# facebookresearch/goliath

Measured on NVIDIA B200. Metric: rendered megapixels/sec (fwd+bwd) RGCA head 300k Gaussians, higher is better.
Workload: dtype f32

## Files before the change

goliath_b200/_lib.py:

```python
import ctypes
import os

import torch

_HERE = os.path.dirname(os.path.abspath(__file__))
LIB_PATH = os.path.join(_HERE, "libgoliath_b200.so")
_lib = None

_vp, _i, _f, _i64, _sz = ctypes.c_void_p, ctypes.c_int, ctypes.c_float, ctypes.c_int64, ctypes.c_size_t

SIGNATURES = {
    "gb_version": (_i, []),
    "gb_launch_count": (ctypes.c_ulonglong, []),
    "gb_launch_count_reset": (None, []),
    "gb_sg_evaluate_fwd": (_i, [_vp] * 7 + [_i] * 4 + [_vp]),
    "gb_sg_evaluate_bwd": (_i, [_vp] * 10 + [_i] * 4 + [_vp]),
    "gb_project_gaussians_fwd": (_i, [_i, _vp, _vp, _f, _vp, _vp, _f, _f, _f, _f, _i, _i, _i, _f] + [_vp] * 7 + [_vp]),
    "gb_project_gaussians_bwd": (_i, [_i, _vp, _vp, _f, _vp, _vp, _f, _f] + [_vp] * 13 + [_vp]),
    "gb_cumsum_workspace_bytes": (_sz, [_i]),
    "gb_cumsum_i32": (_i, [_i, _vp, _vp, _vp, _vp]),
    "gb_map_gaussian_to_intersects": (_i, [_i, _vp, _vp, _vp, _vp, _i, _i, _i, _vp, _vp, _vp]),
    "gb_sort_workspace_bytes": (_sz, [_i64]),
    "gb_sort_intersects": (_i, [_i64, _vp, _vp, _vp, _vp, _i, _vp, _vp]),
    "gb_get_tile_bin_edges": (_i, [_i64, _vp, _vp, _vp]),
    "gb_rasterize_fwd": (_i, [_i, _i, _i, _i] + [_vp] * 10 + [_vp]),
    "gb_rasterize_bwd": (_i, [_i, _i, _i, _i] + [_vp] * 15 + [_vp]),
    "gb_pack_records": (_i, [_i64, _i] + [_vp] * 6 + [_vp]),
    "gb_tile_order": (_i, [_i, _vp, _vp, _vp]),
    "gb_pack_records_fused": (_i, [_i64] + [_vp] * 8 + [_vp]),
    "gb_pack_records_fused_dn": (_i, [_i64] + [_vp] * 9 + [_vp]),
    "gb_map_gaussian_to_intersects_dn": (_i, [_i, _vp, _vp, _vp, _vp, _i, _i, _i, _i64, _vp, _vp, _vp]),
    "gb_sort_intersects_dn": (_i, [_i64, _vp, _vp, _vp, _vp, _vp, _i, _vp, _vp]),
    "gb_get_tile_bin_edges_dn": (_i, [_i64, _vp, _vp, _vp, _vp, _vp]),
    "gb_get_tile_sort_mode": (_i, []),
    "gb_set_tile_sort_mode": (None, [_i]),
    "gb_get_rank_sort_mode": (_i, []),
    "gb_set_rank_sort_mode": (None, [_i]),
    "gb_bin_tiles_supported": (_i, [_i]),
    "gb_bin_tiles_workspace_bytes": (_sz, [_i, _i, _i64]),
    "gb_bin_tiles_pack": (_i, [_i] + [_vp] * 7 + [_i, _i, _i, _i64] + [_vp, _vp, _i] + [_vp] * 5 + [_vp]),
    "gb_bin_tiles_pack_ev": (_i, [_i] + [_vp] * 7 + [_i, _i, _i, _i64] + [_vp, _vp, _i] + [_vp] * 5 + [_vp, _vp]),
    "gb_tile_schedule_ints": (_i, [_i]),
    "gb_tile_schedule": (_i, [_i, _vp, _vp, _vp]),
    "gb_rasterize_sched_fwd": (_i, [_i, _i, _i] + [_vp] * 7 + [_vp]),
    "gb_rasterize_sched_bwd": (_i, [_i, _i, _i] + [_vp] * 13 + [_vp]),
    "gb_records_widen": (_i, [_i64, _vp, _vp, _vp, _vp]),
    "gb_records_set_colors4": (_i, [_i64, _vp, _vp, _vp, _i, _i64, _vp, _vp]),
    "gb_rasterize_multi_fwd": (_i, [_i, _i, _vp, _vp, _i, _vp, _vp, _vp, _vp]),
    "gb_rasterize_multi_bwd": (_i, [_i, _i, _vp, _vp, _vp, _i] + [_vp] * 9 + [_vp]),
    "gb_colors12_unpack": (_i, [_i64, _i, _vp, _vp, _vp]),
    "gb_records_set_colors": (_i, [_i64] + [_vp] * 5 + [_vp]),
    "gb_splat_grad_unpack": (_i, [_i] + [_vp] * 8 + [_vp]),
    "gb_get_blend_mode": (_i, []),
    "gb_set_blend_mode": (None, [_i]),
    "gb_rasterize_packed_fwd": (_i, [_i, _i, _i] + [_vp] * 7 + [_vp]),
    "gb_rasterize_packed_bwd": (_i, [_i, _i, _i] + [_vp] * 13 + [_vp]),
    "gb_rasterize_ranked_fwd": (_i, [_i, _i, _i] + [_vp] * 8 + [_vp]),
    "gb_rasterize_ranked_bwd": (_i, [_i, _i, _i] + [_vp] * 14 + [_vp]),
    "gb_bin_tiles_ranked": (_i, [_i] + [_vp] * 7 + [_i, _i, _i, _i64] + [_vp, _vp, _i] + [_vp] * 6 + [_vp, _vp]),
    "gb_compute_raydirs_fwd": (_i, [_i, _i, _i] + [_vp] * 5 + [_f] + [_vp] * 3 + [_vp]),
    "gb_compute_raydirs_bwd": (_i, []),
    "gb_mvp_aabb_workspace_bytes": (_sz, [_i, _i]),
    "gb_mvp_compute_aabb": (_i, [_i, _i] + [_vp] * 8 + [_vp]),
    "gb_get_raymarch_mode": (_i, []),
    "gb_set_raymarch_mode": (None, [_i]),
    "gb_mvp_raymarch_fwd": (_i, [_i] * 4 + [_vp, _vp, _f] + [_vp] * 5 + [_i] * 3 + [_vp] + [_i] * 3 + [_vp] * 4
# ... 79 lines not shown
```

goliath_b200/csrc/splat_bin_tiles.cu:

```cuda
#include <stdlib.h>
#include <string.h>

#include "common.cuh"
#include "splat_record.cuh"

extern "C" int gb_tile_order(int num_tiles, const int32_t* tile_bins, int32_t* order, void* stream);
extern "C" int gb_tile_schedule(int num_tiles, const int32_t* tile_bins, int32_t* sched, void* stream);
GB_API int gb_bin_tiles_pack_ev(int G, const float* xys, const float* depths, const int32_t* radii, const float* conics,
                                const float* colors3, const float* opacity, const float* compensation, int img_h,
                                int img_w, int block_width, int64_t cap, int32_t* tile_bins, int32_t* tile_order,
                                int tile_sched, int32_t* gids_sorted, float* records, int32_t* n_out, int32_t* overflow,
                                void* workspace, void* colors_ready, void* stream);

namespace {

constexpr int kRankBlock = 256;
constexpr int kRadix = 256;
constexpr int kRankPasses = 4;
constexpr int kScatItems = 2;
constexpr int kSortThreads = 512;
constexpr int kCopyBatch = 2;
constexpr int kMaxBitmapBytes = 192 * 1024;
constexpr int kMaxSmemTiles = 20 * 1024;

// ... 8 lines not shown
    if (lane >= o) inc += t;
  }
  if (lane == 31) s_warp[warp] = inc;
  __syncthreads();
  if (warp == 0) {
    int w = (lane < (int)(blockDim.x >> 5)) ? s_warp[lane] : 0;
    int winc = w;
#pragma unroll
    for (int o = 1; o < 32; o <<= 1) {
      int t = __shfl_up_sync(0xffffffffu, winc, o);
      if (lane >= o) winc += t;
    }
    s_warp[lane] = winc - w;
    if (lane == 31) s_warp[32] = winc;
  }
  __syncthreads();
  total = s_warp[32];
  const int r = s_warp[warp] + inc - v;
  __syncthreads();
  return r;
}

__device__ __forceinline__ void tile_bbox(float cx, float cy, float radius, int tbx, int tby, int bw, int& x0,
                                          int& y0, int& x1, int& y1) {
  const float fb = (float)bw;
  const float tcx = __fdiv_rn(cx, fb), tcy = __fdiv_rn(cy, fb), tr = __fdiv_rn(radius, fb);
  x0 = min(max(0, __float2int_rz(__fsub_rn(tcx, tr))), tbx);
  x1 = min(max(0, __float2int_rz(__fadd_rn(__fadd_rn(tcx, tr), 1.f))), tbx);
  y0 = min(max(0, __float2int_rz(__fsub_rn(tcy, tr))), tby);
  y1 = min(max(0, __float2int_rz(__fadd_rn(__fadd_rn(tcy, tr), 1.f))), tby);
}

constexpr int kGaussBlock = 1024;
template <int kTileKeys>
__global__ void __launch_bounds__(kGaussBlock) depth_keys_kernel(int G, const float2* __restrict__ xys,
                                                                 const float* __restrict__ depths,
                                                                 const int* __restrict__ radii, int tbx, int tby,
                                                                 int block_width, int smem_tiles,
                                                                 unsigned* __restrict__ keys,
                                                                 unsigned* __restrict__ hist0 ,
                                                                 int* __restrict__ tile_counts,
                                                                 unsigned* __restrict__ key_bits ) {
  constexpr int kItems = kTileKeys / kGaussBlock;
  extern __shared__ int s_cnt[];
  __shared__ unsigned s_hist[kRadix];
  __shared__ unsigned s_or, s_orc, s_max, s_maxc;
  if (threadIdx.x == 0) s_or = s_orc = s_max = s_maxc = 0u;
  if (threadIdx.x < kRadix) s_hist[threadIdx.x] = 0;
  for (int t = threadIdx.x; t < smem_tiles; t += kGaussBlock) s_cnt[t] = 0;
  const int base = blockIdx.x * kTileKeys;
  unsigned k[kItems];
  int r[kItems];
  float2 c[kItems];
#pragma unroll
  for (int j = 0; j < kItems; ++j) {
    const int i = base + j * kGaussBlock + threadIdx.x;
    const bool in = i < G;
    k[j] = in ? __float_as_uint(depths[i]) : 0u;
    r[j] = in ? radii[i] : 0;
    c[j] = in ? xys[i] : make_float2(0.f, 0.f);
  }
  {
    unsigned o = 0u, oc = 0u, mx = 0u, mxc = 0u;
#pragma unroll
    for (int j = 0; j < kItems; ++j)
      if (r[j] > 0) { o |= k[j]; oc |= ~k[j]; mx = max(mx, k[j]); mxc = max(mxc, ~k[j]); }
    o = __reduce_or_sync(0xffffffffu, o);
    oc = __reduce_or_sync(0xffffffffu, oc);
    mx = __reduce_max_sync(0xffffffffu, mx);
    mxc = __reduce_max_sync(0xffffffffu, mxc);
    __syncthreads();
    if ((threadIdx.x & 31) == 0 && (o | oc)) {
      atomicOr(&s_or, o); atomicOr(&s_orc, oc); atomicMax(&s_max, mx); atomicMax(&s_maxc, mxc);
    }
  }
  __syncthreads();
#pragma unroll
  for (int j = 0; j < kItems; ++j) {
    const int i = base + j * kGaussBlock + threadIdx.x;
    if (i >= G) continue;
    keys[i] = k[j];
    atomicAdd(&s_hist[k[j] & 0xffu], 1u);
    if (r[j] > 0) {
      int x0, y0, x1, y1;
      tile_bbox(c[j].x, c[j].y, (float)r[j], tbx, tby, block_width, x0, y0, x1, y1);
      for (int ty = y0; ty < y1; ++ty)
        for (int tx = x0; tx < x1; ++tx) {
          if (smem_tiles) atomicAdd(&s_cnt[ty * tbx + tx], 1);
          else atomicAdd(&tile_counts[ty * tbx + tx], 1);
        }
    }
  }
  __syncthreads();
  if (threadIdx.x == 0 && (s_or | s_orc)) {
    atomicOr(key_bits, s_or); atomicOr(key_bits + 1, s_orc);
    atomicMax(key_bits + 4, s_max); atomicMax(key_bits + 5, s_maxc);
  }
  if (threadIdx.x < kRadix) hist0[(size_t)blockIdx.x * kRadix + threadIdx.x] = s_hist[threadIdx.x];
  for (int t = threadIdx.x; t < smem_tiles; t += kGaussBlock) {
    const int cnt = s_cnt[t];
    if (cnt) atomicAdd(&tile_counts[t], cnt);
  }
}

template <int kItems>
__global__ void __launch_bounds__(kRankBlock) rank_scatter_kernel(
    int n, const unsigned* __restrict__ keys_in, const int* __restrict__ vals_in ,
    unsigned* __restrict__ keys_out , int* __restrict__ vals_out, int shift, int ctas,
    const unsigned* __restrict__ hist_cur ,
    unsigned* __restrict__ hist_next ,
    int* __restrict__ rank_of ) {
  constexpr int kWarps = kRankBlock / 32;
  constexpr int kTile = kRankBlock * kItems;
  __shared__ unsigned s_whist[kWarps][kRadix];
  __shared__ int s_scan[33];
  const int lane = threadIdx.x & 31, warp = threadIdx.x >> 5;

  const int warp_base = blockIdx.x * kTile + warp * (32 * kItems);
  unsigned k[kItems];
  int v[kItems];
#pragma unroll
  for (int j = 0; j < kItems; ++j) {
    const int i = warp_base + j * 32 + lane;
    k[j] = (i < n) ? keys_in[i] : 0xffffffffu;
    v[j] = (i < n) ? (vals_in ? vals_in[i] : i) : 0;
  }

  __shared__ uint4 s_part[2][4][kRadix / 4];
  {
    const int g = threadIdx.x >> 6, c4 = threadIdx.x & 63;
    const uint4* tab = reinterpret_cast<const uint4*>(hist_cur);
// ... 356 lines not shown
    for (int j = 0; j < n; ++j) {
      const unsigned kj = s_k[j];
      r += (kj < ki || (kj == ki && s_id[j] < idi)) ? 1 : 0;
    }
    rank_to_gid[off + r] = idi;
    rank_of[idi] = off + r;
  }
}

__global__ void __launch_bounds__(1024) tile_scan_kernel(int T, long long cap, const int* __restrict__ counts,
                                                         int2* __restrict__ tile_bins, int* __restrict__ cursor,
                                                         int* __restrict__ n_out, int* __restrict__ overflow) {
  __shared__ int s_warp[33];
  int carry = 0;
  for (int base = 0; base < T; base += blockDim.x) {
    const int i = base + threadIdx.x;
    const int v = (i < T) ? counts[i] : 0;
    int total;
    const int ex = block_exclusive_scan(v, s_warp, total);
    if (i < T) {
      const int s = carry + ex;
      cursor[i] = s;
      const int cs = (int)min((long long)s, cap), ce = (int)min((long long)s + v, cap);
      tile_bins[i] = (ce > cs) ? make_int2(cs, ce) : make_int2(0, 0);
    }
    carry += total;
  }
  if (threadIdx.x == 0) {
    if (n_out) *n_out = carry;
    if (overflow && (long long)carry > cap) *overflow = 1;
  }
}

__global__ void __launch_bounds__(kGaussBlock) tile_scatter_kernel(
    int G, const float2* __restrict__ xys, const int* __restrict__ radii, const int* __restrict__ rank_of,
    const float* __restrict__ conics, const float* __restrict__ colors3, const float* __restrict__ depths,
    const float* __restrict__ opacity, const float* __restrict__ comp, int tbx, int tby, int block_width,
    long long cap, int smem_tiles, int* __restrict__ cursor, int* __restrict__ tile_ranks,
    float4* __restrict__ rec_by_rank) {
  extern __shared__ int s_cnt[];
  int* s_base = s_cnt + smem_tiles;
  for (int t = threadIdx.x; t < smem_tiles; t += kGaussBlock) s_cnt[t] = 0;
  const int base = blockIdx.x * (kGaussBlock * kScatItems);
  int rk[kScatItems], r[kScatItems];
  float2 c[kScatItems];
#pragma unroll
  for (int j = 0; j < kScatItems; ++j) {
    const int i = base + j * kGaussBlock + threadIdx.x;
    const bool in = i < G;
    r[j] = in ? radii[i] : 0;
    c[j] = in ? xys[i] : make_float2(0.f, 0.f);
    rk[j] = in ? rank_of[i] : 0;
  }
  __syncthreads();
  unsigned bx[kScatItems], by[kScatItems];
#pragma unroll
  for (int j = 0; j < kScatItems; ++j) {
    const int i = base + j * kGaussBlock + threadIdx.x;
    bx[j] = by[j] = 0u;
    if (r[j] <= 0) continue;
    int x0, y0, x1, y1;
    tile_bbox(c[j].x, c[j].y, (float)r[j], tbx, tby, block_width, x0, y0, x1, y1);
    bx[j] = (unsigned)x0 | ((unsigned)x1 << 16);
    by[j] = (unsigned)y0 | ((unsigned)y1 << 16);
    gb::pack_record_fused(i, xys, conics, colors3, depths, opacity, comp, rec_by_rank + 3 * (size_t)rk[j]);
    for (int ty = y0; ty < y1; ++ty)
      for (int tx = x0; tx < x1; ++tx) {
        if (smem_tiles) {
          atomicAdd(&s_cnt[ty * tbx + tx], 1);
        } else {
          const int pos = atomicAdd(&cursor[ty * tbx + tx], 1);
          if ((long long)pos < cap) tile_ranks[pos] = rk[j];
        }
      }
  }
  if (!smem_tiles) return;
  __syncthreads();
  for (int t = threadIdx.x; t < smem_tiles; t += kGaussBlock) {
    const int cnt = s_cnt[t];
    s_base[t] = cnt ? atomicAdd(&cursor[t], cnt) : 0;
    s_cnt[t] = 0;
  }
  __syncthreads();
#pragma unroll
  for (int j = 0; j < kScatItems; ++j) {
    const int x0 = bx[j] & 0xffffu, x1 = bx[j] >> 16, y0 = by[j] & 0xffffu, y1 = by[j] >> 16;
    for (int ty = y0; ty < y1; ++ty)
      for (int tx = x0; tx < x1; ++tx) {
        const int t = ty * tbx + tx;
        const int pos = s_base[t] + atomicAdd(&s_cnt[t], 1);
        if ((long long)pos < cap) tile_ranks[pos] = rk[j];
      }
  }
}

__global__ void __launch_bounds__(kSortThreads, 3) tile_sort_pack_kernel(
    int words , int chunk , const int* __restrict__ order,
    const int2* __restrict__ tile_bins, const int* __restrict__ tile_ranks, const int* __restrict__ rank_to_gid,
    const float4* __restrict__ rec_by_rank, int* __restrict__ gids_sorted, float4* __restrict__ rec) {
  extern __shared__ unsigned s_bits[];
  __shared__ int s_warp[33];
  const int tile = order ? order[blockIdx.x] : (int)blockIdx.x;
  const int2 range = tile_bins[tile];
  const int n = range.y - range.x;
  if (n <= 0) return;
  for (int w = threadIdx.x; w < words; w += kSortThreads) s_bits[w] = 0u;
  __syncthreads();
  for (int i0 = threadIdx.x; i0 < n; i0 += 4 * kSortThreads) {
    int r[4];
#pragma unroll
    for (int u = 0; u < 4; ++u) {
      const int i = i0 + u * kSortThreads;
      r[u] = (i < n) ? tile_ranks[range.x + i] : -1;
    }
#pragma unroll
    for (int u = 0; u < 4; ++u)
      if (r[u] >= 0) atomicOr(&s_bits[r[u] >> 5], 1u << (r[u] & 31));
  }
  __syncthreads();
  const int w0 = threadIdx.x * chunk, w1 = min(words, w0 + chunk);
  int cnt = 0;
  for (int w = w0; w < w1; ++w) cnt += __popc(s_bits[w]);
  int total;
  int pos = range.x + block_exclusive_scan(cnt, s_warp, total);
// ... 43 lines not shown
  const int tile = order ? order[blockIdx.x] : (int)blockIdx.x;
  const int2 range = tile_bins[tile];
  const int n = range.y - range.x;
  if (n <= 0) return;
  for (int w = threadIdx.x; w < words; w += kSortThreads) s_bits[w] = 0u;
  __syncthreads();
  for (int i0 = threadIdx.x; i0 < n; i0 += 4 * kSortThreads) {
    int r[4];
#pragma unroll
    for (int u = 0; u < 4; ++u) {
      const int i = i0 + u * kSortThreads;
      r[u] = (i < n) ? tile_ranks[range.x + i] : -1;
    }
#pragma unroll
    for (int u = 0; u < 4; ++u)
      if (r[u] >= 0) atomicOr(&s_bits[r[u] >> 5], 1u << (r[u] & 31));
  }
  __syncthreads();
  const int w0 = threadIdx.x * chunk, w1 = min(words, w0 + chunk);
  int cnt = 0;
  for (int w = w0; w < w1; ++w) cnt += __popc(s_bits[w]);
  int total;
  int pos = range.x + block_exclusive_scan(cnt, s_warp, total);
  for (int w = w0; w < w1; ++w) {
    unsigned m = s_bits[w];
    while (m) {
      const int b = __ffs(m) - 1;
      m &= m - 1;
      tile_ranks[pos++] = w * 32 + b;
    }
  }
}

__global__ void __launch_bounds__(256) rec_colors_kernel(int G, const int* __restrict__ radii,
                                                         const int* __restrict__ rank_of,
                                                         const float* __restrict__ colors3,
                                                         const float* __restrict__ depths, float4* __restrict__ rec_by_rank) {
  const int g = blockIdx.x * blockDim.x + threadIdx.x;
  if (g >= G || radii[g] <= 0) return;
  rec_by_rank[3 * (size_t)rank_of[g] + 2] = make_float4(colors3[3 * (size_t)g], colors3[3 * (size_t)g + 1],
                                                       colors3[3 * (size_t)g + 2], depths[g]);
}

__global__ void __launch_bounds__(256) gather_records_kernel(long long cap, const int* __restrict__ n_dev,
                                                             const int* __restrict__ ranks_sorted,
                                                             const int* __restrict__ rank_to_gid,
                                                             const float4* __restrict__ rec_by_rank,
                                                             int* __restrict__ gids_sorted, float4* __restrict__ rec) {
  const long long n = min((long long)*n_dev, cap);
  const long long j = (long long)blockIdx.x * blockDim.x + threadIdx.x;
  if (j >= 3 * n) return;
  const long long i = j / 3;
  const int part = (int)(j - 3 * i);
  const int r = ranks_sorted[i];
  rec[j] = gb::ld_nc_f4(rec_by_rank + 3 * (size_t)r + part);
  if (part == 0) gids_sorted[i] = rank_to_gid[r];
}

struct Layout {
  size_t counts, hist, buckets, sync, zero_bytes, cursor, keys_a, keys_b, vals_a, vals_b, rank_to_gid, rank_of, rec_by_rank,
      tile_ranks, total;
};
inline size_t align256(size_t b) { return (b + 255) & ~(size_t)255; }
inline Layout make_layout(int G, int T, int64_t cap) {
  const int g1 = G > 0 ? G : 1;
  const size_t ctas = (size_t)gb::cdiv(g1, kRankBlock * rank_items(g1));
  const size_t g4 = align256((size_t)g1 * 4);
  Layout l;
  size_t o = 0;
  l.counts = o; o += align256((size_t)T * 4);
  l.hist = o;   o += align256(ctas * kRadix * 4 * kRankPasses);
  l.buckets = o; o += align256((size_t)3 * 2048 * 4);
  l.sync = o;   o += 256;
  l.zero_bytes = o;
  l.cursor = o; o += align256((size_t)T * 4);
  l.keys_a = o; o += g4;
  l.keys_b = o; o += g4;
  l.vals_a = o; o += g4;
  l.vals_b = o; o += g4;
  l.rank_to_gid = o; o += g4;
  l.rank_of = o; o += g4;
  l.rec_by_rank = o; o += align256((size_t)g1 * 48);
  l.tile_ranks = o; o += align256((size_t)(cap > 0 ? cap : 1) * 4);
  l.total = o;
  return l;
}

int g_tile_sort_mode = -1;
int tile_sort_mode() {
  if (g_tile_sort_mode < 0) {
    const char* e = getenv("GOLIATH_B200_TILESORT");
    g_tile_sort_mode = (e && strcmp(e, "fused") == 0) ? 1 : 0;
  }
  return g_tile_sort_mode;
}
int g_rank_sort_mode = -1;
int rank_sort_mode() {
  if (g_rank_sort_mode < 0) {
    const char* e = getenv("GOLIATH_B200_RANKSORT");
    g_rank_sort_mode = !e ? 0 : strcmp(e, "passes") == 0 ? 1 : strcmp(e, "buckets") == 0 ? 2 : 0;
  }
  return g_rank_sort_mode;
}
int sm_count() {
  static int n[64] = {};
  int dev = 0;
  if (cudaGetDevice(&dev) != cudaSuccess || dev < 0 || dev >= 64) return gb::kNumSMs;
  if (!n[dev]) {
    int v = 0;
    if (cudaDeviceGetAttribute(&v, cudaDevAttrMultiProcessorCount, dev) != cudaSuccess || v < 1) v = gb::kNumSMs;
    n[dev] = v;
  }
  return n[dev];
}

template <int kItems>
int launch_rank_sort(int G, int ctas, const float* xys, const float* depths, const int32_t* radii, int tbx, int tby,
                     int block_width, int smem_tiles, unsigned* keys_a, unsigned* keys_b, int* vals_a, int* vals_b,
                     unsigned* hist, int* counts, int* buckets, unsigned* sync, int* rank_to_gid, int* rank_of, cudaStream_t s) {
  const size_t hs = (size_t)ctas * kRadix;
  depth_keys_kernel<kRankBlock * kItems><<<ctas, kGaussBlock, (size_t)smem_tiles * 4, s>>>(
      G, (const float2*)xys, depths, radii, tbx, tby, block_width, smem_tiles, keys_a, hist, counts, sync);
  const int mode = rank_sort_mode();
  if (mode == 2) {
    int* bcount = buckets;
    int* boffset = bcount + kBuckets;
    int* bcursor = boffset + kBuckets;
    rank_bucket_count_kernel<kRankBlock * kItems><<<ctas, kGaussBlock, 0, s>>>(G, keys_a, radii, sync, bcount);
    rank_bucket_scan_kernel<<<1, 1024, 0, s>>>(bcount, boffset, bcursor, sync);
    rank_bucket_scatter_kernel<kRankBlock * kItems><<<ctas, kGaussBlock, 0, s>>>(G, keys_a, radii, sync, boffset, bcursor, keys_b,
                                                                               vals_b);
    rank_bucket_sort_kernel<<<kBuckets, kBucketThreads, 0, s>>>(bcount, boffset, sync, keys_b, vals_b, rank_to_gid, rank_of);
    gb::count_launches(4);
  }
  if (mode == 0 || mode == 2) {
    int n = G, tiles = ctas;
    const unsigned* key_bits = sync;
    unsigned* barrier = sync + 2;
    void* args[] = {&n, &tiles, &keys_a, &keys_b, &vals_a, &vals_b, &hist, &key_bits, &barrier, &rank_to_gid, &rank_of};
    const int grid = ctas < sm_count() ? ctas : sm_count();
    if (mode == 2) GB_CUDA(cudaMemsetAsync(sync + 7, 0xff, 4, s));
    GB_CUDA(cudaLaunchCooperativeKernel((const void*)rank_sort_coop_kernel<kItems>, dim3(grid), dim3(kRankBlock), args, 0, s));
    gb::count_launches(2);
    return 0;
  }
  rank_scatter_kernel<kItems><<<ctas, kRankBlock, 0, s>>>(G, keys_a, nullptr, keys_b, vals_b, 0, ctas, hist, hist + hs,
                                                          nullptr);
  rank_scatter_kernel<kItems><<<ctas, kRankBlock, 0, s>>>(G, keys_b, vals_b, keys_a, vals_a, 8, ctas, hist + hs,
                                                          hist + 2 * hs, nullptr);
  rank_scatter_kernel<kItems><<<ctas, kRankBlock, 0, s>>>(G, keys_a, vals_a, keys_b, vals_b, 16, ctas, hist + 2 * hs,
                                                          hist + 3 * hs, nullptr);
  rank_scatter_kernel<kItems><<<ctas, kRankBlock, 0, s>>>(G, keys_b, vals_b, nullptr, rank_to_gid, 24, ctas, hist + 3 * hs,
                                                          nullptr, rank_of);
  gb::count_launches(5);
  return 0;
}

template <typename K>
int opt_in_smem(K kernel, bool* done) {
  int dev = 0;
  GB_CUDA(cudaGetDevice(&dev));
  if (dev < 0 || dev >= 64 || !done[dev]) {
    GB_CUDA(cudaFuncSetAttribute(kernel, cudaFuncAttributeMaxDynamicSharedMemorySize, kMaxBitmapBytes));
    if (dev >= 0 && dev < 64) done[dev] = true;
  }
  return 0;
}

}

GB_API int gb_get_tile_sort_mode(void) { return tile_sort_mode(); }
GB_API void gb_set_tile_sort_mode(int mode) { g_tile_sort_mode = mode ? 1 : 0; }
GB_API int gb_get_rank_sort_mode(void) { return rank_sort_mode(); }
GB_API void gb_set_rank_sort_mode(int mode) { g_rank_sort_mode = mode < 0 ? 0 : (mode > 2 ? 2 : mode); }

GB_API int gb_bin_tiles_supported(int G) { return G >= 1 && ((size_t)gb::cdiv(G, 32) * 4 <= (size_t)kMaxBitmapBytes); }

GB_API size_t gb_bin_tiles_workspace_bytes(int G, int num_tiles, int64_t cap) {
  return make_layout(G, num_tiles, cap).total;
}

GB_API int gb_bin_tiles_pack(int G, const float* xys, const float* depths, const int32_t* radii, const float* conics,
                             const float* colors3, const float* opacity, const float* compensation, int img_h,
                             int img_w, int block_width, int64_t cap, int32_t* tile_bins, int32_t* tile_order,
                             int tile_sched, int32_t* gids_sorted, float* records, int32_t* n_out, int32_t* overflow,
                             void* workspace, void* stream) {
  return gb_bin_tiles_pack_ev(G, xys, depths, radii, conics, colors3, opacity, compensation, img_h, img_w, block_width, cap,
                              tile_bins, tile_order, tile_sched, gids_sorted, records, n_out, overflow, workspace, nullptr,
                              stream);
}

static int bin_tiles_impl(int G, const float* xys, const float* depths, const int32_t* radii, const float* conics,
                          const float* colors3, const float* opacity, const float* compensation, int img_h, int img_w,
                          int block_width, int64_t cap, int32_t* tile_bins, int32_t* tile_order, int tile_sched,
                          int32_t* gids_sorted, float* records, int32_t* n_out, int32_t* overflow, void* workspace,
                          void* colors_ready, void* stream, int32_t* ext_ranks, float* ext_rec, int32_t* ext_r2g);

GB_API int gb_bin_tiles_pack_ev(int G, const float* xys, const float* depths, const int32_t* radii, const float* conics,
                                const float* colors3, const float* opacity, const float* compensation, int img_h,
                                int img_w, int block_width, int64_t cap, int32_t* tile_bins, int32_t* tile_order,
                                int tile_sched, int32_t* gids_sorted, float* records, int32_t* n_out, int32_t* overflow,
                                void* workspace, void* colors_ready, void* stream) {
  return bin_tiles_impl(G, xys, depths, radii, conics, colors3, opacity, compensation, img_h, img_w, block_width, cap,
// ... 10 lines not shown
  return bin_tiles_impl(G, xys, depths, radii, conics, colors3, opacity, compensation, img_h, img_w, block_width, cap,
                        tile_bins, tile_order, tile_sched, nullptr, nullptr, n_out, overflow, workspace, colors_ready, stream,
                        ranks_sorted, rec_by_rank, rank_to_gid);
}

static int bin_tiles_impl(int G, const float* xys, const float* depths, const int32_t* radii, const float* conics,
                          const float* colors3, const float* opacity, const float* compensation, int img_h, int img_w,
                          int block_width, int64_t cap, int32_t* tile_bins, int32_t* tile_order, int tile_sched,
                          int32_t* gids_sorted, float* records, int32_t* n_out, int32_t* overflow, void* workspace,
                          void* colors_ready, void* stream, int32_t* ext_ranks, float* ext_rec, int32_t* ext_r2g) {
  if (!gb_bin_tiles_supported(G) || block_width < 1 || cap < 0) return (int)cudaErrorInvalidValue;
  cudaStream_t s = (cudaStream_t)stream;
  const int tbx = gb::cdiv(img_w, block_width), tby = gb::cdiv(img_h, block_width);
  const int T = tbx * tby;
  if (T < 1 || tbx > 65535 || tby > 65535) return (int)cudaErrorInvalidValue;
  const Layout l = make_layout(G, T, cap);
  char* ws = (char*)workspace;
  int* counts = (int*)(ws + l.counts);
  unsigned* hist = (unsigned*)(ws + l.hist);
  int* cursor = (int*)(ws + l.cursor);
  unsigned* keys_a = (unsigned*)(ws + l.keys_a);
  unsigned* keys_b = (unsigned*)(ws + l.keys_b);
  int* vals_a = (int*)(ws + l.vals_a);
  int* vals_b = (int*)(ws + l.vals_b);
  const bool ranked = ext_ranks != nullptr;
  int* rank_to_gid = ranked ? ext_r2g : (int*)(ws + l.rank_to_gid);
  unsigned* sync = (unsigned*)(ws + l.sync);
  int* rank_of = (int*)(ws + l.rank_of);
  float4* rec_by_rank = ranked ? (float4*)ext_rec : (float4*)(ws + l.rec_by_rank);
  int* tile_ranks = ranked ? ext_ranks : (int*)(ws + l.tile_ranks);
  const int items = rank_items(G);
  const int ctas = gb::cdiv(G, kRankBlock * items);
  const int smem_tiles = (T <= kMaxSmemTiles) ? T : 0;
  static bool s_opt_k8[64] = {}, s_opt_k16[64] = {}, s_opt_scat[64] = {}, s_opt_sort[64] = {}, s_opt_sort2[64] = {};
  if ((size_t)smem_tiles * 8 > 40 * 1024) {
    int e = (items == 8) ? opt_in_smem(depth_keys_kernel<kRankBlock * 8>, s_opt_k8)
                         : opt_in_smem(depth_keys_kernel<kRankBlock * 16>, s_opt_k16);
    if (e) return e;
    e = opt_in_smem(tile_scatter_kernel, s_opt_scat);
    if (e) return e;
  }

  GB_CUDA(cudaMemsetAsync(ws, 0, l.zero_bytes, s));
  const int es = (items == 8)
                     ? launch_rank_sort<8>(G, ctas, xys, depths, radii, tbx, tby, block_width, smem_tiles, keys_a, keys_b,
                                           vals_a, vals_b, hist, counts, (int*)(ws + l.buckets), sync, rank_to_gid, rank_of, s)
                     : launch_rank_sort<16>(G, ctas, xys, depths, radii, tbx, tby, block_width, smem_tiles, keys_a, keys_b,
                                            vals_a, vals_b, hist, counts, (int*)(ws + l.buckets), sync, rank_to_gid, rank_of, s);
  if (es) return es;
  int* n_total = n_out ? n_out : (int*)(sync + 3);
  tile_scan_kernel<<<1, 1024, 0, s>>>(T, (long long)cap, counts, (int2*)tile_bins, cursor, n_total, overflow);
  gb::count_launches(1);
  GB_CHECK_LAUNCH();
  const int e = tile_sched ? gb_tile_schedule(T, tile_bins, tile_order, stream)
                           : gb_tile_order(T, tile_bins, tile_order, stream);
  if (e) return e;
  const bool split = ranked || tile_sort_mode() == 0;
  const bool late = split && colors_ready;
  if (!late && colors_ready) GB_CUDA(cudaStreamWaitEvent(s, (cudaEvent_t)colors_ready, 0));
  tile_scatter_kernel<<<gb::cdiv(G, kGaussBlock * kScatItems), kGaussBlock, (size_t)smem_tiles * 8, s>>>(
      G, (const float2*)xys, radii, rank_of, conics, late ? nullptr : colors3, depths, opacity, compensation, tbx, tby,
      block_width, (long long)cap, smem_tiles, cursor, tile_ranks, rec_by_rank);
  const int words = gb::cdiv(G, 32);
  const int chunk = gb::cdiv(words, kSortThreads) | 1;
  const size_t smem = (size_t)words * 4;
  if (split) {
    if (smem > 40 * 1024) {
      const int e2 = opt_in_smem(tile_sort_kernel, s_opt_sort2);
      if (e2) return e2;
    }
    tile_sort_kernel<<<T, kSortThreads, smem, s>>>(words, chunk, tile_order, (const int2*)tile_bins, tile_ranks);
    if (late) {
      GB_CUDA(cudaStreamWaitEvent(s, (cudaEvent_t)colors_ready, 0));
      rec_colors_kernel<<<gb::cdiv(G, 256), 256, 0, s>>>(G, radii, rank_of, colors3, depths, rec_by_rank);
      gb::count_launches(1);
    }
    if (cap > 0 && !ranked)
      gather_records_kernel<<<(unsigned)gb::cdiv64(3 * cap, 256), 256, 0, s>>>((long long)cap, n_total, tile_ranks, rank_to_gid,
                                                                             rec_by_rank, gids_sorted, (float4*)records);
    gb::count_launches(3);
    GB_CHECK_LAUNCH();
    return 0;
  }
  if (smem > 40 * 1024) {
    const int e2 = opt_in_smem(tile_sort_pack_kernel, s_opt_sort);
    if (e2) return e2;
  }
  tile_sort_pack_kernel<<<T, kSortThreads, smem, s>>>(words, chunk, tile_order, (const int2*)tile_bins, tile_ranks,
                                                      rank_to_gid, rec_by_rank, gids_sorted, (float4*)records);
  gb::count_launches(2);
  GB_CHECK_LAUNCH();
  return 0;
}
```

include/goliath_b200.h:

```cpp
#ifndef GOLIATH_B200_H_
#define GOLIATH_B200_H_

#include <stddef.h>
#include <stdint.h>

#ifdef __cplusplus
extern "C" {
#endif

int gb_version(void);
unsigned long long gb_launch_count(void);
void gb_launch_count_reset(void);


int gb_sg_evaluate_fwd(const float* lobe_dirs, const float* lobe_sigmas, const float* light_values,
                       const float* light_pts, const float* prim_pts, const int32_t* n_lights, float* integral,
                       int N, int D, int L, int w_type, void* stream);

int gb_sg_evaluate_bwd(const float* lobe_dirs, const float* lobe_sigmas, const float* light_values,
                       const float* light_pts, const float* prim_pts, const int32_t* n_lights,
                       const float* grad_integral, float* grad_dirs, float* grad_sigmas, float* grad_light_values,
                       int N, int D, int L, int w_type, void* stream);


// ... 41 lines not shown
int gb_pack_records_fused(int64_t n, const int32_t* gids_sorted, const float* xys, const float* conics,
                          const float* colors3, const float* depths, const float* opacity, const float* compensation,
                          float* records, void* stream);

int gb_records_set_colors(int64_t cap, const int32_t* n_dev, const int32_t* gids_sorted, const float* colors3,
                          const float* depths, float* records, void* stream);

int gb_records_widen(int64_t cap, const int32_t* n_dev, const float* records, float* records_wide, void* stream);
int gb_records_set_colors4(int64_t cap, const int32_t* n_dev, const int32_t* gids_sorted, const float* colors, int nk,
                           int64_t G, float* records_wide, void* stream);
int gb_rasterize_multi_fwd(int img_h, int img_w, const int32_t* tile_bins, const int32_t* tile_order, int sched,
                           const float* records_wide, const float* background, float* out_planes, void* stream);
int gb_rasterize_multi_bwd(int img_h, int img_w, const int32_t* gids_sorted, const int32_t* tile_bins,
                           const int32_t* tile_order, int sched, const float* records_wide, const float* background,
                           const float* final_Ts, const int32_t* final_idx, const float* v_planes, float* v_xy, float* v_conic,
                           float* v_colors12, float* v_opacity, void* stream);
int gb_colors12_unpack(int64_t G, int nk, float* v_colors12, float* v_colors, void* stream);

int gb_splat_grad_unpack(int G, const float* v_colors4, const float* v_opac_eff, const float* opacity,
                         const float* compensation, float* v_colors3, float* v_opacity, float* v_comp, float* v_depth,
                         void* stream);

int gb_map_gaussian_to_intersects_dn(int G, const float* xys, const float* depths, const int32_t* radii,
                                     const int32_t* cum_tiles_hit, int img_h, int img_w, int block_width, int64_t cap,
                                     int64_t* isect_ids, int32_t* gaussian_ids, void* stream);
int gb_sort_intersects_dn(int64_t cap, const int32_t* n_dev, const int64_t* isect_ids, const int32_t* gaussian_ids,
                          int64_t* isect_sorted, int32_t* gids_sorted, int key_bits, void* workspace, void* stream);
int gb_get_tile_bin_edges_dn(int64_t cap, const int32_t* n_dev, const int64_t* isect_sorted, int32_t* tile_bins,
                             int32_t* overflow, void* stream);
int gb_pack_records_fused_dn(int64_t cap, const int32_t* n_dev, const int32_t* gids_sorted, const float* xys,
                             const float* conics, const float* colors3, const float* depths, const float* opacity,
                             const float* compensation, float* records, void* stream);

int gb_get_rank_sort_mode(void);
int gb_get_tile_sort_mode(void);
void gb_set_tile_sort_mode(int mode);
void gb_set_rank_sort_mode(int mode);

int gb_bin_tiles_supported(int G);
size_t gb_bin_tiles_workspace_bytes(int G, int num_tiles, int64_t cap);
int gb_bin_tiles_pack(int G, const float* xys, const float* depths, const int32_t* radii, const float* conics,
                      const float* colors3, const float* opacity, const float* compensation, int img_h, int img_w,
                      int block_width, int64_t cap, int32_t* tile_bins, int32_t* tile_order, int tile_sched,
                      int32_t* gids_sorted, float* records, int32_t* n_out, int32_t* overflow, void* workspace,
                      void* stream);
int gb_bin_tiles_pack_ev(int G, const float* xys, const float* depths, const int32_t* radii, const float* conics,
                         const float* colors3, const float* opacity, const float* compensation, int img_h, int img_w,
                         int block_width, int64_t cap, int32_t* tile_bins, int32_t* tile_order, int tile_sched,
                         int32_t* gids_sorted, float* records, int32_t* n_out, int32_t* overflow, void* workspace,
                         void* colors_ready, void* stream);

int gb_bin_tiles_ranked(int G, const float* xys, const float* depths, const int32_t* radii, const float* conics,
                        const float* colors3, const float* opacity, const float* compensation, int img_h, int img_w,
                        int block_width, int64_t cap, int32_t* tile_bins, int32_t* tile_order, int tile_sched,
                        int32_t* ranks_sorted, float* rec_by_rank, int32_t* rank_to_gid, int32_t* n_out, int32_t* overflow,
                        void* workspace, void* colors_ready, void* stream);
int gb_rasterize_ranked_fwd(int img_h, int img_w, int channels, const int32_t* tile_bins, const int32_t* tile_order,
                            const int32_t* ranks_sorted, const float* rec_by_rank, const float* background,
                            float* out_img, float* final_Ts, int32_t* final_idx, void* stream);
int gb_rasterize_ranked_bwd(int img_h, int img_w, int channels, const int32_t* rank_to_gid, const int32_t* ranks_sorted,
                            const int32_t* tile_bins, const int32_t* tile_order, const float* rec_by_rank,
                            const float* background, const float* final_Ts, const int32_t* final_idx,
                            const float* v_output, const float* v_output_alpha, float* v_xy, float* v_conic,
                            float* v_colors, float* v_opacity, void* stream);

int gb_tile_order(int num_tiles, const int32_t* tile_bins, int32_t* order, void* stream);
// ... 161 lines not shown
```

Before: 1708.

## Replace global depth rank sort with per-tile key/id pair radix sort

Adds a default bin-sort mode that skips the global radix sort over Gaussian depth keys. Each tile slot now stores the raw depth bits and the Gaussian id, and a new per-tile kernel sorts the (depth, id) pairs in shared memory, falling back to the records buffer as scratch for large tiles. Records are packed by Gaussian id and gathered in sorted order. This removes several global sort passes, at the cost of per-tile sorting work that is uneven across tiles, so heavy tiles can dominate.

```diff
diff --git a/goliath_b200/_lib.py b/goliath_b200/_lib.py
--- a/goliath_b200/_lib.py
+++ b/goliath_b200/_lib.py
@@ -32,6 +32,8 @@
     "gb_map_gaussian_to_intersects_dn": (_i, [_i, _vp, _vp, _vp, _vp, _i, _i, _i, _i64, _vp, _vp, _vp]),
     "gb_sort_intersects_dn": (_i, [_i64, _vp, _vp, _vp, _vp, _vp, _i, _vp, _vp]),
     "gb_get_tile_bin_edges_dn": (_i, [_i64, _vp, _vp, _vp, _vp, _vp]),
+    "gb_get_bin_sort_mode": (_i, []),
+    "gb_set_bin_sort_mode": (None, [_i]),
     "gb_get_tile_sort_mode": (_i, []),
     "gb_set_tile_sort_mode": (None, [_i]),
     "gb_get_rank_sort_mode": (_i, []),
diff --git a/goliath_b200/csrc/splat_bin_tiles.cu b/goliath_b200/csrc/splat_bin_tiles.cu
--- a/goliath_b200/csrc/splat_bin_tiles.cu
+++ b/goliath_b200/csrc/splat_bin_tiles.cu
@@ -64,7 +64,7 @@
 }
 
 constexpr int kGaussBlock = 1024;
-template <int kTileKeys>
+template <int kTileKeys, bool kRank>
 __global__ void __launch_bounds__(kGaussBlock) depth_keys_kernel(int G, const float2* __restrict__ xys,
                                                                  const float* __restrict__ depths,
                                                                  const int* __restrict__ radii, int tbx, int tby,
@@ -111,8 +111,10 @@
   for (int j = 0; j < kItems; ++j) {
     const int i = base + j * kGaussBlock + threadIdx.x;
     if (i >= G) continue;
-    keys[i] = k[j];
-    atomicAdd(&s_hist[k[j] & 0xffu], 1u);
+    if (kRank) {
+      keys[i] = k[j];
+      atomicAdd(&s_hist[k[j] & 0xffu], 1u);
+    }
     if (r[j] > 0) {
       int x0, y0, x1, y1;
       tile_bbox(c[j].x, c[j].y, (float)r[j], tbx, tby, block_width, x0, y0, x1, y1);
@@ -128,7 +130,7 @@
     atomicOr(key_bits, s_or); atomicOr(key_bits + 1, s_orc);
     atomicMax(key_bits + 4, s_max); atomicMax(key_bits + 5, s_maxc);
   }
-  if (threadIdx.x < kRadix) hist0[(size_t)blockIdx.x * kRadix + threadIdx.x] = s_hist[threadIdx.x];
+  if (kRank && threadIdx.x < kRadix) hist0[(size_t)blockIdx.x * kRadix + threadIdx.x] = s_hist[threadIdx.x];
   for (int t = threadIdx.x; t < smem_tiles; t += kGaussBlock) {
     const int cnt = s_cnt[t];
     if (cnt) atomicAdd(&tile_counts[t], cnt);
@@ -551,11 +553,12 @@
   }
 }
 
+template <bool kById>
 __global__ void __launch_bounds__(kGaussBlock) tile_scatter_kernel(
     int G, const float2* __restrict__ xys, const int* __restrict__ radii, const int* __restrict__ rank_of,
     const float* __restrict__ conics, const float* __restrict__ colors3, const float* __restrict__ depths,
     const float* __restrict__ opacity, const float* __restrict__ comp, int tbx, int tby, int block_width,
-    long long cap, int smem_tiles, int* __restrict__ cursor, int* __restrict__ tile_ranks,
+    long long cap, int smem_tiles, int* __restrict__ cursor, int* __restrict__ tile_ranks, int* __restrict__ slot_ids,
     float4* __restrict__ rec_by_rank) {
   extern __shared__ int s_cnt[];
   int* s_base = s_cnt + smem_tiles;
@@ -569,7 +572,8 @@
     const bool in = i < G;
     r[j] = in ? radii[i] : 0;
     c[j] = in ? xys[i] : make_float2(0.f, 0.f);
-    rk[j] = in ? rank_of[i] : 0;
+    if (kById) rk[j] = in ? __float_as_int(depths[i]) : 0;
+    else rk[j] = in ? rank_of[i] : 0;
   }
   __syncthreads();
   unsigned bx[kScatItems], by[kScatItems];
@@ -582,14 +586,17 @@
     tile_bbox(c[j].x, c[j].y, (float)r[j], tbx, tby, block_width, x0, y0, x1, y1);
     bx[j] = (unsigned)x0 | ((unsigned)x1 << 16);
     by[j] = (unsigned)y0 | ((unsigned)y1 << 16);
-    gb::pack_record_fused(i, xys, conics, colors3, depths, opacity, comp, rec_by_rank + 3 * (size_t)rk[j]);
+    gb::pack_record_fused(i, xys, conics, colors3, depths, opacity, comp, rec_by_rank + 3 * (size_t)(kById ? i : rk[j]));
     for (int ty = y0; ty < y1; ++ty)
       for (int tx = x0; tx < x1; ++tx) {
         if (smem_tiles) {
           atomicAdd(&s_cnt[ty * tbx + tx], 1);
         } else {
           const int pos = atomicAdd(&cursor[ty * tbx + tx], 1);
-          if ((long long)pos < cap) tile_ranks[pos] = rk[j];
+          if ((long long)pos < cap) {
+            tile_ranks[pos] = rk[j];
+            if (kById) slot_ids[pos] = i;
+          }
         }
       }
   }
@@ -608,7 +615,10 @@
       for (int tx = x0; tx < x1; ++tx) {
         const int t = ty * tbx + tx;
         const int pos = s_base[t] + atomicAdd(&s_cnt[t], 1);
-        if ((long long)pos < cap) tile_ranks[pos] = rk[j];
+        if ((long long)pos < cap) {
+          tile_ranks[pos] = rk[j];
+          if (kById) slot_ids[pos] = base + j * kGaussBlock + threadIdx.x;
+        }
       }
   }
 }
@@ -718,21 +728,164 @@
   }
 }
 
+constexpr int kPairThreads = 512;
+constexpr int kPairWarps = kPairThreads / 32;
+constexpr int kPairCap = 6144;
+constexpr size_t kPairSmem = (size_t)2 * kPairCap * 8 + (size_t)kPairWarps * kRadix * 4;
+
+__device__ __forceinline__ unsigned long long* pair_radix_sort(unsigned long long* a, unsigned long long* b, int n,
+                                                               unsigned long long varying, unsigned* s_hist, int* s_warp) {
+  const int lane = threadIdx.x & 31, warp = threadIdx.x >> 5;
+  const int per = (n + kPairWarps - 1) / kPairWarps;
+  const int c0 = min(n, warp * per), c1 = min(n, c0 + per);
+  const unsigned lt = (1u << lane) - 1u;
+  unsigned* h = s_hist + warp * kRadix;
+  for (int shift = 0; shift < 64; shift += 8) {
+    if (((varying >> shift) & 0xffull) == 0ull) continue;
+    for (int d = lane; d < kRadix; d += 32) h[d] = 0u;
+    __syncwarp();
+    for (int i = c0 + lane; i < c1; i += 32) atomicAdd(&h[(unsigned)(a[i] >> shift) & 0xffu], 1u);
+    __syncthreads();
+    {
+      const int d = threadIdx.x;
+      unsigned tot = 0u;
+      if (d < kRadix)
+        for (int w = 0; w < kPairWarps; ++w) tot += s_hist[w * kRadix + d];
+      int unused;
+      unsigned run = (unsigned)block_exclusive_scan((int)tot, s_warp, unused);
+      if (d < kRadix)
+        for (int w = 0; w < kPairWarps; ++w) {
+          const unsigned c = s_hist[w * kRadix + d];
+          s_hist[w * kRadix + d] = run;
+          run += c;
+        }
+    }
+    __syncthreads();
+    for (int i0 = c0; i0 < c1; i0 += 32) {
+      const int i = i0 + lane;
+      const bool valid = i < c1;
+      const unsigned long long v = valid ? a[i] : 0ull;
+      const unsigned dg = valid ? ((unsigned)(v >> shift) & 0xffu) : 0x100u;
+      const unsigned peers = __match_any_sync(0xffffffffu, dg);
+      const unsigned lower = peers & lt;
+      const unsigned at = valid ? h[dg] : 0u;
+      __syncwarp();
+      if (valid) {
+        b[at + __popc(lower)] = v;
+        if (lower == 0u) h[dg] = at + __popc(peers);
+      }
+      __syncwarp();
+    }
+    __syncthreads();
+    unsigned long long* t = a;
+    a = b;
+    b = t;
+  }
+  return a;
+}
+
+constexpr int kMaxRun = 32;
+__device__ __forceinline__ void pair_sort_tile(unsigned long long* a, unsigned long long* b, int2 range,
+                                               unsigned kmin, const unsigned* __restrict__ tile_keys,
+                                               int* __restrict__ gids_sorted, unsigned* s_hist, int* s_warp,
+                                               unsigned long long* s_or_and) {
+  const int n = range.y - range.x;
+  unsigned long long o = 0ull, an = ~0ull;
+  for (int i0 = threadIdx.x; i0 < n; i0 += 4 * kPairThreads) {
+    unsigned k[4];
+    int g[4];
+#pragma unroll
+    for (int u = 0; u < 4; ++u) {
+      const int i = i0 + u * kPairThreads;
+      k[u] = (i < n) ? tile_keys[range.x + i] : kmin;
+      g[u] = (i < n) ? gids_sorted[range.x + i] : 0;
+    }
+#pragma unroll
+    for (int u = 0; u < 4; ++u) {
+      const int i = i0 + u * kPairThreads;
+      if (i < n) {
+        const unsigned long long c = ((unsigned long long)(k[u] - kmin) << 32) | (unsigned)g[u];
+        a[i] = c;
+        o |= c;
+        an &= c;
+      }
+    }
+  }
+  const unsigned olo = __reduce_or_sync(0xffffffffu, (unsigned)o), ohi = __reduce_or_sync(0xffffffffu, (unsigned)(o >> 32));
+  const unsigned alo = __reduce_and_sync(0xffffffffu, (unsigned)an),
+                 ahi = __reduce_and_sync(0xffffffffu, (unsigned)(an >> 32));
+  if ((threadIdx.x & 31) == 0) {
+    atomicOr(&s_or_and[0], ((unsigned long long)ohi << 32) | olo);
+    atomicAnd(&s_or_and[1], ((unsigned long long)ahi << 32) | alo);
+  }
+  __syncthreads();
+  const unsigned long long varying = s_or_and[0] & ~s_or_and[1];
+  unsigned long long* res = pair_radix_sort(a, b, n, varying & 0xffffffff00000000ull, s_hist, s_warp);
+  bool long_run = false;
+  for (int i = threadIdx.x; i < n; i += kPairThreads) {
+    const unsigned key = (unsigned)(res[i] >> 32);
+    if (i > 0 && (unsigned)(res[i - 1] >> 32) == key) continue;
+    int e = i + 1;
+    while (e < n && e - i <= kMaxRun && (unsigned)(res[e] >> 32) == key) ++e;
+    if (e - i > kMaxRun) {
+      long_run = true;
+    } else {
+      for (int j = i + 1; j < e; ++j) {
+        const unsigned long long v = res[j];
+        int p = j - 1;
+        while (p >= i && res[p] > v) {
+          res[p + 1] = res[p];
+          --p;
+        }
+        res[p + 1] = v;
+      }
+    }
+  }
+  if (__syncthreads_or(long_run)) res = pair_radix_sort(res, res == a ? b : a, n, varying, s_hist, s_warp);
+  for (int i = threadIdx.x; i < n; i += kPairThreads) gids_sorted[range.x + i] = (int)(unsigned)res[i];
+}
+
+__global__ void __launch_bounds__(kPairThreads, 2) tile_pair_sort_kernel(
+    const int* __restrict__ order, const int2* __restrict__ tile_bins,
+    const unsigned* __restrict__ key_bits , const unsigned* __restrict__ tile_keys,
+    int* __restrict__ gids_sorted, float* __restrict__ records ) {
+  extern __shared__ unsigned long long s_pairs[];
+  __shared__ int s_warp[33];
+  __shared__ unsigned long long s_or_and[2];
+  const int tile = order ? order[blockIdx.x] : (int)blockIdx.x;
+  const int2 range = tile_bins[tile];
+  const int n = range.y - range.x;
+  if (n <= 1) return;
+  if (threadIdx.x == 0) {
+    s_or_and[0] = 0ull;
+    s_or_and[1] = ~0ull;
+  }
+  __syncthreads();
+  const unsigned kmin = ~key_bits[5];
+  unsigned* s_hist = reinterpret_cast<unsigned*>(s_pairs + 2 * kPairCap);
+  if (n <= kPairCap) {
+    pair_sort_tile(s_pairs, s_pairs + kPairCap, range, kmin, tile_keys, gids_sorted, s_hist, s_warp, s_or_and);
+  } else {
+    unsigned long long* a = reinterpret_cast<unsigned long long*>(records + 12 * (size_t)range.x);
+    pair_sort_tile(a, a + n, range, kmin, tile_keys, gids_sorted, s_hist, s_warp, s_or_and);
+  }
+}
+
 __global__ void __launch_bounds__(256) rec_colors_kernel(int G, const int* __restrict__ radii,
                                                          const int* __restrict__ rank_of,
                                                          const float* __restrict__ colors3,
                                                          const float* __restrict__ depths, float4* __restrict__ rec_by_rank) {
   const int g = blockIdx.x * blockDim.x + threadIdx.x;
   if (g >= G || radii[g] <= 0) return;
-  rec_by_rank[3 * (size_t)rank_of[g] + 2] = make_float4(colors3[3 * (size_t)g], colors3[3 * (size_t)g + 1],
-                                                       colors3[3 * (size_t)g + 2], depths[g]);
+  const size_t at = rank_of ? (size_t)rank_of[g] : (size_t)g;
+  rec_by_rank[3 * at + 2] = make_float4(colors3[3 * (size_t)g], colors3[3 * (size_t)g + 1], colors3[3 * (size_t)g + 2],
+                                        depths[g]);
 }
 
 __global__ void __launch_bounds__(256) gather_records_kernel(long long cap, const int* __restrict__ n_dev,
-                                                             const int* __restrict__ ranks_sorted,
-                                                             const int* __restrict__ rank_to_gid,
-                                                             const float4* __restrict__ rec_by_rank,
-                                                             int* __restrict__ gids_sorted, float4* __restrict__ rec) {
+                                                             const int* ranks_sorted, const int* __restrict__ rank_to_gid,
+                                                             const float4* __restrict__ rec_by_rank, int* gids_sorted,
+                                                             float4* __restrict__ rec) {
   const long long n = min((long long)*n_dev, cap);
   const long long j = (long long)blockIdx.x * blockDim.x + threadIdx.x;
   if (j >= 3 * n) return;
@@ -740,7 +893,7 @@
   const int part = (int)(j - 3 * i);
   const int r = ranks_sorted[i];
   rec[j] = gb::ld_nc_f4(rec_by_rank + 3 * (size_t)r + part);
-  if (part == 0) gids_sorted[i] = rank_to_gid[r];
+  if (rank_to_gid && part == 0) gids_sorted[i] = rank_to_gid[r];
 }
 
 struct Layout {
@@ -780,6 +933,14 @@
   }
   return g_tile_sort_mode;
 }
+int g_bin_sort_mode = -1;
+int bin_sort_mode() {
+  if (g_bin_sort_mode < 0) {
+    const char* e = getenv("GOLIATH_B200_BINSORT");
+    g_bin_sort_mode = (e && strcmp(e, "rank") == 0) ? 1 : 0;
+  }
+  return g_bin_sort_mode;
+}
 int g_rank_sort_mode = -1;
 int rank_sort_mode() {
   if (g_rank_sort_mode < 0) {
@@ -805,7 +966,7 @@
                      int block_width, int smem_tiles, unsigned* keys_a, unsigned* keys_b, int* vals_a, int* vals_b,
                      unsigned* hist, int* counts, int* buckets, unsigned* sync, int* rank_to_gid, int* rank_of, cudaStream_t s) {
   const size_t hs = (size_t)ctas * kRadix;
-  depth_keys_kernel<kRankBlock * kItems><<<ctas, kGaussBlock, (size_t)smem_tiles * 4, s>>>(
+  depth_keys_kernel<kRankBlock * kItems, true><<<ctas, kGaussBlock, (size_t)smem_tiles * 4, s>>>(
       G, (const float2*)xys, depths, radii, tbx, tby, block_width, smem_tiles, keys_a, hist, counts, sync);
   const int mode = rank_sort_mode();
   if (mode == 2) {
@@ -855,6 +1016,8 @@
 
 }
 
+GB_API int gb_get_bin_sort_mode(void) { return bin_sort_mode(); }
+GB_API void gb_set_bin_sort_mode(int mode) { g_bin_sort_mode = mode ? 1 : 0; }
 GB_API int gb_get_tile_sort_mode(void) { return tile_sort_mode(); }
 GB_API void gb_set_tile_sort_mode(int mode) { g_tile_sort_mode = mode ? 1 : 0; }
 GB_API int gb_get_rank_sort_mode(void) { return rank_sort_mode(); }
@@ -931,22 +1094,36 @@
   const int items = rank_items(G);
   const int ctas = gb::cdiv(G, kRankBlock * items);
   const int smem_tiles = (T <= kMaxSmemTiles) ? T : 0;
+  const bool by_id = !ranked && bin_sort_mode() == 0;
   static bool s_opt_k8[64] = {}, s_opt_k16[64] = {}, s_opt_scat[64] = {}, s_opt_sort[64] = {}, s_opt_sort2[64] = {};
+  static bool s_opt_k8i[64] = {}, s_opt_k16i[64] = {}, s_opt_scati[64] = {}, s_opt_pair[64] = {};
   if ((size_t)smem_tiles * 8 > 40 * 1024) {
-    int e = (items == 8) ? opt_in_smem(depth_keys_kernel<kRankBlock * 8>, s_opt_k8)
-                         : opt_in_smem(depth_keys_kernel<kRankBlock * 16>, s_opt_k16);
+    int e = by_id ? ((items == 8) ? opt_in_smem(depth_keys_kernel<kRankBlock * 8, false>, s_opt_k8i)
+                                  : opt_in_smem(depth_keys_kernel<kRankBlock * 16, false>, s_opt_k16i))
+                  : ((items == 8) ? opt_in_smem(depth_keys_kernel<kRankBlock * 8, true>, s_opt_k8)
+                                  : opt_in_smem(depth_keys_kernel<kRankBlock * 16, true>, s_opt_k16));
     if (e) return e;
-    e = opt_in_smem(tile_scatter_kernel, s_opt_scat);
+    e = by_id ? opt_in_smem(tile_scatter_kernel<true>, s_opt_scati) : opt_in_smem(tile_scatter_kernel<false>, s_opt_scat);
     if (e) return e;
   }
 
   GB_CUDA(cudaMemsetAsync(ws, 0, l.zero_bytes, s));
-  const int es = (items == 8)
-                     ? launch_rank_sort<8>(G, ctas, xys, depths, radii, tbx, tby, block_width, smem_tiles, keys_a, keys_b,
-                                           vals_a, vals_b, hist, counts, (int*)(ws + l.buckets), sync, rank_to_gid, rank_of, s)
-                     : launch_rank_sort<16>(G, ctas, xys, depths, radii, tbx, tby, block_width, smem_tiles, keys_a, keys_b,
-                                            vals_a, vals_b, hist, counts, (int*)(ws + l.buckets), sync, rank_to_gid, rank_of, s);
-  if (es) return es;
+  if (by_id) {
+    if (items == 8)
+      depth_keys_kernel<kRankBlock * 8, false><<<ctas, kGaussBlock, (size_t)smem_tiles * 4, s>>>(
+          G, (const float2*)xys, depths, radii, tbx, tby, block_width, smem_tiles, nullptr, nullptr, counts, sync);
+    else
+      depth_keys_kernel<kRankBlock * 16, false><<<ctas, kGaussBlock, (size_t)smem_tiles * 4, s>>>(
+          G, (const float2*)xys, depths, radii, tbx, tby, block_width, smem_tiles, nullptr, nullptr, counts, sync);
+    gb::count_launches(1);
+  } else {
+    const int es = (items == 8)
+                       ? launch_rank_sort<8>(G, ctas, xys, depths, radii, tbx, tby, block_width, smem_tiles, keys_a, keys_b,
+                                             vals_a, vals_b, hist, counts, (int*)(ws + l.buckets), sync, rank_to_gid, rank_of, s)
+                       : launch_rank_sort<16>(G, ctas, xys, depths, radii, tbx, tby, block_width, smem_tiles, keys_a, keys_b,
+                                              vals_a, vals_b, hist, counts, (int*)(ws + l.buckets), sync, rank_to_gid, rank_of, s);
+    if (es) return es;
+  }
   int* n_total = n_out ? n_out : (int*)(sync + 3);
   tile_scan_kernel<<<1, 1024, 0, s>>>(T, (long long)cap, counts, (int2*)tile_bins, cursor, n_total, overflow);
   gb::count_launches(1);
@@ -954,12 +1131,35 @@
   const int e = tile_sched ? gb_tile_schedule(T, tile_bins, tile_order, stream)
                            : gb_tile_order(T, tile_bins, tile_order, stream);
   if (e) return e;
-  const bool split = ranked || tile_sort_mode() == 0;
+  const bool split = by_id || ranked || tile_sort_mode() == 0;
   const bool late = split && colors_ready;
   if (!late && colors_ready) GB_CUDA(cudaStreamWaitEvent(s, (cudaEvent_t)colors_ready, 0));
-  tile_scatter_kernel<<<gb::cdiv(G, kGaussBlock * kScatItems), kGaussBlock, (size_t)smem_tiles * 8, s>>>(
+  const int scat_ctas = gb::cdiv(G, kGaussBlock * kScatItems);
+  if (by_id) {
+    tile_scatter_kernel<true><<<scat_ctas, kGaussBlock, (size_t)smem_tiles * 8, s>>>(
+        G, (const float2*)xys, radii, nullptr, conics, late ? nullptr : colors3, depths, opacity, compensation, tbx, tby,
+        block_width, (long long)cap, smem_tiles, cursor, tile_ranks, gids_sorted, rec_by_rank);
+    if (cap > 0) {
+      const int e2 = opt_in_smem(tile_pair_sort_kernel, s_opt_pair);
+      if (e2) return e2;
+      tile_pair_sort_kernel<<<T, kPairThreads, kPairSmem, s>>>(tile_order, (const int2*)tile_bins, sync,
+                                                               (const unsigned*)tile_ranks, gids_sorted, records);
+    }
+    if (late) {
+      GB_CUDA(cudaStreamWaitEvent(s, (cudaEvent_t)colors_ready, 0));
+      rec_colors_kernel<<<gb::cdiv(G, 256), 256, 0, s>>>(G, radii, nullptr, colors3, depths, rec_by_rank);
+      gb::count_launches(1);
+    }
+    if (cap > 0)
+      gather_records_kernel<<<(unsigned)gb::cdiv64(3 * cap, 256), 256, 0, s>>>((long long)cap, n_total, gids_sorted, nullptr,
+                                                                               rec_by_rank, gids_sorted, (float4*)records);
+    gb::count_launches(3);
+    GB_CHECK_LAUNCH();
+    return 0;
+  }
+  tile_scatter_kernel<false><<<scat_ctas, kGaussBlock, (size_t)smem_tiles * 8, s>>>(
       G, (const float2*)xys, radii, rank_of, conics, late ? nullptr : colors3, depths, opacity, compensation, tbx, tby,
-      block_width, (long long)cap, smem_tiles, cursor, tile_ranks, rec_by_rank);
+      block_width, (long long)cap, smem_tiles, cursor, tile_ranks, nullptr, rec_by_rank);
   const int words = gb::cdiv(G, 32);
   const int chunk = gb::cdiv(words, kSortThreads) | 1;
   const size_t smem = (size_t)words * 4;
diff --git a/include/goliath_b200.h b/include/goliath_b200.h
--- a/include/goliath_b200.h
+++ b/include/goliath_b200.h
@@ -97,6 +97,8 @@
                              const float* conics, const float* colors3, const float* depths, const float* opacity,
                              const float* compensation, float* records, void* stream);
 
+int gb_get_bin_sort_mode(void);
+void gb_set_bin_sort_mode(int mode);
 int gb_get_rank_sort_mode(void);
 int gb_get_tile_sort_mode(void);
 void gb_set_tile_sort_mode(int mode);
```

Result: faster. 1799, median of 6 (+5.3%).
